# ray-project/kuberay

Measured on AMD Instinct MI355X. Metric: rayclusters_to_ready_per_sec, higher is better.
Workload: dtype bf16; 1 GPU; model=raycluster-control-plane, global_batch=2500, seq_len=4, parallelism=dp1, workers_per_cluster=3, gpus_per_worker=1, kubelet=simulated (envtest methodology; no real kubelet)

## Files before the change

### kuberay_amd/_native/build.py

```python
from __future__ import annotations

import os
import subprocess
import sys
import sysconfig
from pathlib import Path

HERE = Path(__file__).resolve().parent
GFX_ARCH = os.environ.get("PYTORCH_ROCM_ARCH", "gfx950")
HIPCC = os.environ.get("HIPCC", "/opt/rocm/bin/hipcc")


def _ext_suffix() -> str:
    return sysconfig.get_config_var("EXT_SUFFIX") or ".so"


def _pybind11_includes() -> list:
    import pybind11
    return [f"-I{pybind11.get_include()}",
            f"-I{sysconfig.get_paths()['include']}"]


def _needs_rebuild(src: Path, out: Path, *deps: Path) -> bool:
    if not out.exists():
# ... 11 lines not shown
        HIPCC, f"--offload-arch={GFX_ARCH}", "-O3", "-std=c++17",
        "-shared", "-fPIC", *_pybind11_includes(),
        str(src), "-o", str(out),
    ]
    subprocess.run(cmd, check=True)
    return out


def build_engine(force: bool = False) -> Path:
    src = HERE / "engine.cpp"
    out = HERE / f"engine{_ext_suffix()}"
    if not src.exists():
        return out
    if not force and not _needs_rebuild(src, out, HERE / "store_core.hpp",
                                        HERE / "tree_copy.hpp",
                                        HERE / "json_decode.hpp"):
        return out
    cxx = os.environ.get("CXX", "g++")
    cmd = [
        cxx, "-O3", "-std=c++17", "-shared", "-fPIC",
        *_pybind11_includes(), str(src), "-o", str(out),
    ]
    subprocess.run(cmd, check=True)
    return out


def build_all(force: bool = False) -> list:
    outs = [build_gpuhealth(force)]
    if (HERE / "engine.cpp").exists():
        outs.append(build_engine(force))
    return outs
# ... 7 lines not shown
```

### kuberay_amd/_native/engine.cpp

```cpp

#include <pybind11/pybind11.h>
#include <pybind11/stl.h>

#include <cmath>
#include <cstdio>
#include <optional>
#include <string>
#include <unordered_set>
#include <vector>

#define KUBERAY_JSON_WITH_PYTHON
#include "json_decode.hpp"
#include "store_core.hpp"
#include "tree_copy.hpp"

namespace py = pybind11;
using namespace kuberay_store;

namespace {

struct Decline {};

constexpr int kMaxDepth = 128;

struct Keys {
  PyObject *metadata, *status, *spec, *labels, *ownerReferences, *uid,
      *resourceVersion, *finalizers, *deletionTimestamp, *name, *ns, *phase,
      *podIP, *restartPolicy, *creationTimestamp, *conditions, *type,
      *containers, *containerStatuses, *state, *terminated, *clusterIP, *ports,
      *port, *nodePort;
};
Keys K;

void init_keys() {
  auto mk = [](const char* s) { return PyUnicode_InternFromString(s); };
  K.metadata = mk("metadata"); K.status = mk("status"); K.spec = mk("spec");
  K.labels = mk("labels"); K.ownerReferences = mk("ownerReferences");
  K.uid = mk("uid"); K.resourceVersion = mk("resourceVersion");
  K.finalizers = mk("finalizers");
  K.deletionTimestamp = mk("deletionTimestamp");
  K.name = mk("name"); K.ns = mk("namespace"); K.phase = mk("phase");
  K.podIP = mk("podIP"); K.restartPolicy = mk("restartPolicy");
  K.creationTimestamp = mk("creationTimestamp");
  K.conditions = mk("conditions"); K.type = mk("type");
  K.containers = mk("containers");
  K.containerStatuses = mk("containerStatuses"); K.state = mk("state");
  K.terminated = mk("terminated");
  K.clusterIP = mk("clusterIP"); K.ports = mk("ports"); K.port = mk("port");
  K.nodePort = mk("nodePort");
}


void encode_str(PyObject* s, std::string& out) {
  Py_ssize_t n = 0;
  const char* p = PyUnicode_AsUTF8AndSize(s, &n);
  if (p == nullptr) {
    PyErr_Clear();
    throw Decline{};
  }
  static const char* hex = "0123456789abcdef";
  out.push_back('"');
  const char* run = p;
  const char* end = p + n;
  for (const char* c = p; c < end; ++c) {
// ... 275 lines not shown
using ServiceViewTuple =
    std::tuple<std::string, std::string, std::string, std::vector<PortTuple>>;

Section make_section(const std::string& scratch) {
  return std::make_shared<const std::string>(scratch.data(), scratch.size());
}

py::bytes to_bytes(const Blob& b) {
  const size_t n = b.size();
  PyObject* out = PyBytes_FromStringAndSize(nullptr, static_cast<Py_ssize_t>(n));
  if (out == nullptr) throw py::error_already_set();
  b.write(PyBytes_AS_STRING(out));
  return py::reinterpret_steal<py::bytes>(out);
}

class NativeStore {
 public:
  explicit NativeStore(size_t history_capacity) : core_(history_capacity) {}

  py::object put_object(const std::string& kind, const std::string& ns,
                        const std::string& name, py::handle obj,
                        const std::optional<std::string>& event_type) {
    static thread_local std::string rest, meta_s, status_s;
    rest.clear(); meta_s.clear(); status_s.clear();
    Blob blob;
    Fields f;
    try {
      PyObject* o = obj.ptr();
      if (!PyDict_CheckExact(o)) throw Decline{};
      bool has_meta = false, has_status = false;
      Py_ssize_t pos = 0;
      PyObject *k, *v;
      while (PyDict_Next(o, &pos, &k, &v)) {
        if (!PyUnicode_CheckExact(k)) throw Decline{};
        if (PyUnicode_CompareWithASCIIString(k, "metadata") == 0) {
          encode(v, meta_s, 1);
          has_meta = true;
        } else if (PyUnicode_CompareWithASCIIString(k, "status") == 0) {
          encode(v, status_s, 1);
          has_status = true;
        } else {
          if (!rest.empty()) rest.push_back(',');
          encode_str(k, rest);
// ... 7 lines not shown
      f.rv = std::move(p.rv); f.uid = std::move(p.uid);
      f.deletion_ts = std::move(p.deletion_ts);
      f.has_finalizers = p.has_finalizers;
      extract_indexes(meta, f);
      if (kind == "Pod") {
        extract_view(o, meta, f.view);
        f.has_view = true;
      } else if (kind == "Service") {
        f.has_service_view = extract_service_view(o, meta, f.service_view);
      }
      blob.rest = make_section(rest);
      if (has_meta) blob.meta = make_section(meta_s);
      if (has_status) blob.status = make_section(status_s);
    } catch (const Decline&) {
      core_.note_fallback();
      return py::none();
    }
    core_.note_encode(true, rest.size() + meta_s.size() + status_s.size());
    const bool is_new = core_.put(kind, ns, name, std::move(blob), std::move(f),
                                  event_type ? event_type->c_str() : nullptr);
    return py::bool_(is_new);
  }

  py::object put_status(const std::string& kind, const std::string& ns,
                        const std::string& name, py::handle obj,
                        const std::optional<std::string>& event_type) {
    static thread_local std::string meta_s, status_s;
    meta_s.clear(); status_s.clear();
    Section meta_sec, status_sec;
    Peek p;
    PodViewData view;
    const bool is_pod = kind == "Pod";
    try {
      PyObject* o = obj.ptr();
      if (!PyDict_CheckExact(o)) throw Decline{};
      PyObject* meta = metadata_of(o);
      if (meta != nullptr) {
        encode(meta, meta_s, 1);
        meta_sec = make_section(meta_s);
      }
      if (PyObject* status = dget(o, K.status)) {
        encode(status, status_s, 1);
        status_sec = make_section(status_s);
      }
      extract_peek(meta, p);
      if (is_pod) extract_view(o, meta, view);
    } catch (const Decline&) {
      return py::none();
    }
    if (!core_.put_status(kind, ns, name, std::move(meta_sec),
                          std::move(status_sec), std::move(p), is_pod,
                          std::move(view),
                          event_type ? event_type->c_str() : nullptr)) {
      return py::none();
    }
    core_.note_encode(false, meta_s.size() + status_s.size());
    return py::bool_(true);
  }

  bool put(const std::string& kind, const std::string& ns,
           const std::string& name, const std::string& blob,
           const std::string& rv, const LabelList& labels,
           const std::vector<std::string>& owner_uids,
           const std::optional<PodViewData>& view,
           const std::optional<std::string>& event_type,
           const std::string& uid, bool has_finalizers,
           const std::string& deletion_ts,
           const std::optional<ServiceViewTuple>& service_view) {
    Blob b;
    b.rest = std::make_shared<const std::string>(blob);
    b.whole = true;
    Fields f;
// ... 203 lines not shown

  std::vector<int64_t> history_rvs() const { return core_.history_rvs(); }

  py::dict stats() const {
    const Stats s = core_.stats();
    py::dict d;
    d["full_encodes"] = s.full_encodes;
    d["partial_encodes"] = s.partial_encodes;
    d["bytes_encoded"] = s.bytes_encoded;
    d["blobs_assembled"] = s.blobs_assembled;
    d["bytes_assembled"] = s.bytes_assembled;
    d["fallbacks"] = s.fallbacks;
    d["history_appends"] = s.history_appends;
    d["trees_decoded"] = s.trees_decoded;
    d["decode_fallbacks"] = s.decode_fallbacks;
    return d;
  }

 private:
  StoreCore core_;
};

}

PYBIND11_MODULE(engine, m) {
  m.doc() = "kuberay-amd native object store (C++ sections + indexes + pod "
            "and Service views + watch history, native JSON encoding) and "
            "model-tree copier";
  init_keys();

  m.def("copy_configure", [](py::handle base_model) {
    return kuberay_copy::configure(base_model.ptr());
  }, py::arg("base_model"),
        "Hand the copier pydantic.BaseModel; returns whether it is enabled.");
  m.def("copy_tree", [](py::handle obj) -> py::object {
// ... 10 lines not shown
    return d;
  });

  py::class_<PodViewData>(m, "PodViewData")
      .def(py::init<>())
      .def_readwrite("name", &PodViewData::name)
      .def_readwrite("ns", &PodViewData::ns)
      .def_readwrite("phase", &PodViewData::phase)
      .def_readwrite("deletion_ts", &PodViewData::deletion_ts)
      .def_readwrite("pod_ip", &PodViewData::pod_ip)
      .def_readwrite("restart_policy", &PodViewData::restart_policy)
      .def_readwrite("creation_ts", &PodViewData::creation_ts)
      .def_readwrite("ready", &PodViewData::ready)
      .def_readwrite("terminated", &PodViewData::terminated);

  py::class_<NativeStore>(m, "NativeStore")
      .def(py::init<size_t>(), py::arg("history_capacity") = 1024)
      .def("put_object", &NativeStore::put_object, py::arg("kind"),
           py::arg("ns"), py::arg("name"), py::arg("obj"),
           py::arg("event_type") = std::nullopt)
      .def("put_status", &NativeStore::put_status, py::arg("kind"),
           py::arg("ns"), py::arg("name"), py::arg("obj"),
           py::arg("event_type") = std::nullopt)
      .def("put", &NativeStore::put, py::arg("kind"), py::arg("ns"),
           py::arg("name"), py::arg("blob"), py::arg("rv"), py::arg("labels"),
           py::arg("owner_uids"), py::arg("view") = std::nullopt,
           py::arg("event_type") = std::nullopt, py::arg("uid") = "",
           py::arg("has_finalizers") = false, py::arg("deletion_ts") = "",
           py::arg("service_view") = std::nullopt)
      .def("fetch", &NativeStore::fetch)
      .def("fetch_tree", &NativeStore::fetch_tree)
      .def("remove_tree", &NativeStore::remove_tree, py::arg("kind"),
// ... 27 lines not shown
```

### kuberay_amd/_native/store_core.hpp

```cpp
#pragma once

#include <algorithm>
#include <atomic>
#include <cstdint>
#include <cstring>
#include <memory>
#include <mutex>
#include <optional>
#include <string>
#include <tuple>
#include <unordered_map>
#include <unordered_set>
#include <utility>
#include <vector>

namespace kuberay_store {

using Section = std::shared_ptr<const std::string>;
using LabelList = std::vector<std::pair<std::string, std::string>>;

struct PodViewData {
  std::string name, ns, phase, deletion_ts, pod_ip, restart_policy, creation_ts;
  bool ready = false;
  bool terminated = false;
// ... 77 lines not shown
  PodViewData view;
  LabelList labels;
};

struct HistoryItem {
  std::string event_type;
  Blob blob;
  std::optional<int64_t> rv_override;
};

struct Stats {
  uint64_t full_encodes = 0, partial_encodes = 0, bytes_encoded = 0;
  uint64_t blobs_assembled = 0, bytes_assembled = 0;
  uint64_t fallbacks = 0, history_appends = 0;
  uint64_t trees_decoded = 0, decode_fallbacks = 0;
};

inline std::string make_key(const std::string& kind, const std::string& ns,
                            const std::string& name) {
  std::string k;
  k.reserve(kind.size() + ns.size() + name.size() + 2);
  k += kind; k += '\x1f'; k += ns; k += '\x1f'; k += name;
  return k;
}

inline std::string label_key(const std::string& kind, const std::string& k,
                             const std::string& v) {
  std::string out;
  out.reserve(kind.size() + k.size() + v.size() + 2);
  out += kind; out += '\x1f'; out += k; out += '\x1f'; out += v;
// ... 63 lines not shown
    return it->second.f.rv;
  }

  std::optional<Peek> peek(const std::string& kind, const std::string& ns,
                           const std::string& name) const {
    std::lock_guard<std::mutex> g(mu_);
    auto it = objects_.find(make_key(kind, ns, name));
    if (it == objects_.end()) return std::nullopt;
    const Fields& f = it->second.f;
    Peek p;
    p.rv = f.rv; p.uid = f.uid; p.deletion_ts = f.deletion_ts;
    p.has_finalizers = f.has_finalizers;
    return p;
  }

  bool contains(const std::string& kind, const std::string& ns,
                const std::string& name) const {
    std::lock_guard<std::mutex> g(mu_);
    return objects_.count(make_key(kind, ns, name)) != 0;
  }

  std::optional<Blob> remove(const std::string& kind, const std::string& ns,
                             const std::string& name,
                             std::optional<int64_t> event_rv = std::nullopt) {
    std::lock_guard<std::mutex> g(mu_);
    auto it = objects_.find(make_key(kind, ns, name));
    if (it == objects_.end()) return std::nullopt;
    Blob out = std::move(it->second.blob);
    index_remove(it->first, it->second);
    objects_.erase(it);
// ... 128 lines not shown

  void note_encode(bool full, size_t bytes) {
    (full ? full_encodes_ : partial_encodes_).fetch_add(1, std::memory_order_relaxed);
    bytes_encoded_.fetch_add(bytes, std::memory_order_relaxed);
  }
  void note_assembled(size_t blobs, size_t bytes) {
    blobs_assembled_.fetch_add(blobs, std::memory_order_relaxed);
    bytes_assembled_.fetch_add(bytes, std::memory_order_relaxed);
  }
  void note_fallback() { fallbacks_.fetch_add(1, std::memory_order_relaxed); }
  void note_decode(bool decoded) {
    (decoded ? trees_decoded_ : decode_fallbacks_)
        .fetch_add(1, std::memory_order_relaxed);
  }

  Stats stats() const {
    Stats s;
    s.full_encodes = full_encodes_.load(std::memory_order_relaxed);
    s.partial_encodes = partial_encodes_.load(std::memory_order_relaxed);
    s.bytes_encoded = bytes_encoded_.load(std::memory_order_relaxed);
    s.blobs_assembled = blobs_assembled_.load(std::memory_order_relaxed);
    s.bytes_assembled = bytes_assembled_.load(std::memory_order_relaxed);
    s.fallbacks = fallbacks_.load(std::memory_order_relaxed);
    s.history_appends = history_appends_.load(std::memory_order_relaxed);
    s.trees_decoded = trees_decoded_.load(std::memory_order_relaxed);
    s.decode_fallbacks = decode_fallbacks_.load(std::memory_order_relaxed);
    return s;
  }

 private:
  struct Entry {
    std::string kind, ns, name;
// ... 113 lines not shown
  mutable std::mutex mu_;
  std::unordered_map<std::string, Entry> objects_;
  std::unordered_map<std::string, std::unordered_set<std::string>> kind_index_;
  std::unordered_map<std::string, std::unordered_set<std::string>> label_index_;
  std::unordered_map<std::string, std::unordered_set<std::string>> owner_index_;

  std::vector<HistEntry> ring_;
  size_t ring_head_ = 0, ring_len_ = 0;
  int64_t base_ = 0;
  int64_t last_rv_ = 0;

  std::atomic<uint64_t> full_encodes_{0}, partial_encodes_{0}, bytes_encoded_{0};
  std::atomic<uint64_t> blobs_assembled_{0}, bytes_assembled_{0};
  std::atomic<uint64_t> fallbacks_{0}, history_appends_{0};
  std::atomic<uint64_t> trees_decoded_{0}, decode_fallbacks_{0};
};

}
```

### kuberay_amd/kube/controller.py

```python
from __future__ import annotations

import dataclasses
import logging
import threading
import traceback
from typing import Any, Dict, List, Optional, Tuple

from .store import ConflictError, InMemoryApiServer
from .workqueue import RateLimitingQueue

logger = logging.getLogger("kuberay.controller")

Request = Tuple[str, str]


@dataclasses.dataclass
class Result:
    requeue: bool = False
    requeue_after: Optional[float] = None


class Reconciler:

    def reconcile(self, request: Request) -> Result:
# ... 133 lines not shown


class Manager:

    def __init__(self, server: InMemoryApiServer):
        self.server = server
        self.controllers: List[Controller] = []
        self._watcher = None
        self._thread: Optional[threading.Thread] = None
        self._stopped = threading.Event()

    def add_controller(self, controller: Controller) -> None:
        self.controllers.append(controller)

    def _dispatch_loop(self) -> None:
        while not self._stopped.is_set():
            ev = self._watcher.next(timeout=0.5)
            if ev is None:
                continue
            event_type, obj = ev
            for c in self.controllers:
                c.observe(event_type, obj)

    def start(self) -> None:
        kinds = set()
        for c in self.controllers:
            kinds.add(c.primary_kind)
            kinds.update(c.owned_kinds)
        self._watcher = self.server.watch(kinds)
        for c in self.controllers:
            for obj in self.server.list(c.primary_kind):
                c.observe("ADDED", obj)
        self._thread = threading.Thread(target=self._dispatch_loop,
                                        name="manager-dispatch", daemon=True)
        self._thread.start()
        for c in self.controllers:
            c.start()

    def stop(self) -> None:
        self._stopped.set()
        for c in self.controllers:
            c.stop()
        if self._watcher:
# ... 13 lines not shown
```

### kuberay_amd/kube/kubelet.py

```python
from __future__ import annotations

import heapq
import itertools
import threading
import time
from typing import Callable, List, Optional, Tuple

from ..utils import constants as C
from .store import InMemoryApiServer, NotFoundError, now_iso


class SimKubelet:
    def __init__(
        self,
        server: InMemoryApiServer,
        startup_delay: float = 0.0,
        job_runtime: float = 0.05,
        gpu_gate: Optional[Callable[[dict], bool]] = None,
        executors: int = 1,
    ):
        self.server = server
        self.startup_delay = startup_delay
        self.job_runtime = job_runtime
        self.gpu_gate = gpu_gate
        self.executors = max(1, executors)
        self._ip_counter = itertools.count(1)
        self._timer_lock = threading.Condition()
        self._timers: List[Tuple[float, int, Callable[[], None]]] = []
        self._seq = 0
        self._stopped = threading.Event()
        self._threads: List[threading.Thread] = []
        self._watcher = None

    WATCHED_KINDS = ("Pod", "Job", "Gateway", "HTTPRoute")

    def start(self) -> None:
        self._watcher = self.server.watch(set(self.WATCHED_KINDS))
        for kind in self.WATCHED_KINDS:
            for obj in self.server.list(kind):
                self._on_event("ADDED", obj)
        t1 = threading.Thread(target=self._watch_loop, name="sim-kubelet-watch", daemon=True)
        self._threads = [t1]
        for i in range(self.executors):
            self._threads.append(threading.Thread(
                target=self._timer_loop, name=f"sim-kubelet-timer-{i}",
                daemon=True))
        for t in self._threads:
            t.start()

    def stop(self) -> None:
        self._stopped.set()
        if self._watcher:
# ... 158 lines not shown
```

### kuberay_amd/kube/native.py

```python
from __future__ import annotations

import json
import os
from typing import Any, Dict, List, Optional, Tuple

from .._native import engine
from .store import Key, PodView, ServiceView, compute_service_view

_dumps = json.dumps
_loads = json.loads


def _view_of(obj: Dict[str, Any]):
    status = obj.get("status") or {}
    spec = obj.get("spec") or {}
    meta = obj.get("metadata", {})
    v = engine.PodViewData()
    v.name = meta.get("name", "")
    v.ns = meta.get("namespace", "default")
    v.phase = status.get("phase") or ""
    v.deletion_ts = meta.get("deletionTimestamp") or ""
    v.pod_ip = status.get("podIP") or ""
    v.restart_policy = spec.get("restartPolicy") or ""
    v.creation_ts = meta.get("creationTimestamp") or ""
# ... 5 lines not shown
        ray_name = containers[0].get("name")
        for cs in status.get("containerStatuses") or []:
            if cs.get("name") == ray_name and (cs.get("state") or {}).get("terminated"):
                v.terminated = True
                break
    return v


class NativeBackend:
    name = "native-cpp"

    native_encode = os.environ.get("KUBERAY_STORE_NATIVE_ENCODE", "1") != "0"
    status_splice = os.environ.get("KUBERAY_STORE_STATUS_SPLICE", "1") != "0"
    native_decode = os.environ.get("KUBERAY_STORE_NATIVE_DECODE", "1") != "0"

    def __init__(self, history_limit: int = 1024) -> None:
        self._store = engine.NativeStore(history_limit)
        self._kind_counts: Dict[str, int] = {}

    def put(self, key: Key, obj: Dict[str, Any],
            event_type: Optional[str] = None) -> None:
        kind, ns, name = key
        is_new = (self._store.put_object(kind, ns, name, obj, event_type)
                  if self.native_encode else None)
        if is_new is None:
            is_new = self._put_blob(key, obj, event_type)
        if is_new:
            self._kind_counts[kind] = self._kind_counts.get(kind, 0) + 1

    def _put_blob(self, key: Key, obj: Dict[str, Any],
                  event_type: Optional[str]) -> bool:
        kind, ns, name = key
        meta = obj.get("metadata", {})
# ... 127 lines not shown
```

### kuberay_amd/kube/store.py

```python
from __future__ import annotations

import dataclasses
import threading
import time
import uuid
from collections import defaultdict, deque
from typing import Any, Dict, Iterable, List, Optional, Tuple

Key = Tuple[str, str, str]


def jsoncopy(obj):
    t = type(obj)
    if t is dict:
        return {k: jsoncopy(v) for k, v in obj.items()}
    if t is list:
        return [jsoncopy(v) for v in obj]
    return obj


class ApiError(Exception):
    def __init__(self, code: int, message: str):
        super().__init__(f"{code}: {message}")
        self.code = code
# ... 7 lines not shown

class ConflictError(ApiError):
    def __init__(self, message: str = "conflict"):
        super().__init__(409, message)


class AlreadyExistsError(ApiError):
    def __init__(self, message: str = "already exists"):
        super().__init__(409, message)


class GoneError(ApiError):

    def __init__(self, message: str = "resource version too old"):
        super().__init__(410, message)


def now_iso() -> str:
    return time.strftime("%Y-%m-%dT%H:%M:%SZ", time.gmtime())


def match_labels(labels: Optional[Dict[str, str]], selector: Optional[Dict[str, str]]) -> bool:
    if not selector:
        return True
    labels = labels or {}
    return all(labels.get(k) == v for k, v in selector.items())



@dataclasses.dataclass
# ... 217 lines not shown
class InMemoryApiServer:

    EVENT_HISTORY_LIMIT = 1024

    def __init__(self, backend=None) -> None:
        self._lock = threading.RLock()
        self._backend = backend if backend is not None else default_backend()
        self._rv = 0
        self._watchers: List["Watcher"] = []
        self._event_history: deque = deque(maxlen=self.EVENT_HISTORY_LIMIT)
        self._history_base: int = 0
        self._fast = all(hasattr(self._backend, n) for n in (
            "put_status", "peek", "history_since", "history_reset"))
        if self._fast:
            self._backend.history_reset(0, self.EVENT_HISTORY_LIMIT)

    @property
    def backend_name(self) -> str:
        return self._backend.name

    def _next_rv(self) -> str:
        self._rv += 1
        return str(self._rv)

    def _put(self, key: Key, obj: Dict[str, Any], event_type: str,
             status_only: bool = False) -> None:
        if not self._fast:
            self._backend.put(key, obj)
        elif status_only:
            self._backend.put_status(key, obj, event_type)
        else:
            self._backend.put(key, obj, event_type)

    def _notify(self, event_type: str, obj: Dict[str, Any]) -> None:
        if not self._fast:
            try:
                rv = int(obj.get("metadata", {}).get("resourceVersion") or self._rv)
            except (TypeError, ValueError):
                rv = self._rv
            if event_type == "DELETED":
                rv = self._rv
            import json as _json
            self._event_history.append(
                (rv, event_type, obj.get("kind", ""),
                 _json.dumps(obj, separators=(",", ":"))))
        for w in list(self._watchers):
            w.push(event_type, obj)

    def reset_history(self, rv: int) -> None:
        with self._lock:
            self._rv = rv
            self._history_base = rv
            self._event_history.clear()
            if self._fast:
                self._backend.history_reset(rv, self.EVENT_HISTORY_LIMIT)

    @property
    def current_rv(self) -> int:
        with self._lock:
            return self._rv
# ... 18 lines not shown
        return (obj.get("kind", ""), meta.get("namespace", "default"),
                meta.get("name", ""))

    def create(self, obj: Dict[str, Any], *, assume_owned: bool = False) -> Dict[str, Any]:
        if not assume_owned:
            obj = jsoncopy(obj)
        meta = obj.setdefault("metadata", {})
        meta.setdefault("namespace", "default")
        if not meta.get("name"):
            gen = meta.get("generateName")
            if not gen:
                raise ApiError(422, "name or generateName required")
            meta["name"] = gen + uuid.uuid4().hex[:5]
        with self._lock:
            key = self._key_of(obj)
            if self._backend.contains(key):
                raise AlreadyExistsError(f"{key} already exists")
            meta["uid"] = str(uuid.uuid4())
            meta["resourceVersion"] = self._next_rv()
            meta["generation"] = 1
            meta["creationTimestamp"] = now_iso()
            self._put(key, obj, "ADDED")
        self._notify("ADDED", obj)
        return obj

    def get(self, kind: str, namespace: str, name: str) -> Dict[str, Any]:
        with self._lock:
            obj = self._backend.fetch((kind, namespace, name))
        if obj is None:
            raise NotFoundError(f"{kind} {namespace}/{name} not found")
        return obj

    def try_get(self, kind: str, namespace: str, name: str) -> Optional[Dict[str, Any]]:
        with self._lock:
            return self._backend.fetch((kind, namespace, name))

# ... 13 lines not shown
            return self._backend.list_views(namespace, label_selector)

    def service_view(self, namespace: str, name: str) -> Optional[ServiceView]:
        fn = getattr(self._backend, "service_view", None)
        if fn is None:
            return None
        with self._lock:
            return fn(("Service", namespace, name))

    def update(self, obj: Dict[str, Any], *, subresource: Optional[str] = None,
               assume_owned: bool = False) -> Dict[str, Any]:
        if not assume_owned:
            obj = jsoncopy(obj)
        key = self._key_of(obj)
        with self._lock:
            current = self._backend.fetch(key)
            if current is None:
                raise NotFoundError(f"{key} not found")
            new_obj, finalizers_gone = self._apply_update(
                key, obj, current, subresource)
        self._notify("MODIFIED", new_obj)
        if finalizers_gone:
            self._finalize_delete(key)
        return new_obj

    def _apply_update(self, key: Key, obj: Dict[str, Any],
                      current: Dict[str, Any], subresource: Optional[str]):
        meta = obj.setdefault("metadata", {})
        rv = meta.get("resourceVersion")
        cur_meta = current["metadata"]
        if rv is not None and rv != cur_meta["resourceVersion"]:
            raise ConflictError(
                f"{key}: resourceVersion mismatch {rv} != {cur_meta['resourceVersion']}")
        if subresource == "status":
            new_obj = current
            new_obj["status"] = obj.get("status", {})
# ... 53 lines not shown
                key, merged, current, subresource)
        self._notify("MODIFIED", new_obj)
        if finalizers_gone:
            self._finalize_delete(key)
        return new_obj

    def mutate_status(self, kind: str, namespace: str, name: str,
                      fn) -> Optional[Dict[str, Any]]:
        key = (kind, namespace, name)
        with self._lock:
            obj = self._backend.fetch(key)
            if obj is None:
                return None
            if fn(obj) is False:
                return None
            new_obj, finalizers_gone = self._apply_update(
                key, obj, obj, "status")
        self._notify("MODIFIED", new_obj)
        if finalizers_gone:
            self._finalize_delete(key)
        return new_obj

    def delete(self, kind: str, namespace: str, name: str) -> None:
        key = (kind, namespace, name)
        with self._lock:
            if self._fast:
                peeked = self._backend.peek(key)
                if peeked is None:
                    raise NotFoundError(f"{kind} {namespace}/{name} not found")
                _, _, has_finalizers, deletion_ts = peeked
                if has_finalizers and deletion_ts:
                    return
                current = self._backend.fetch(key) if has_finalizers else None
            else:
                current = self._backend.fetch(key)
                if current is None:
                    raise NotFoundError(f"{kind} {namespace}/{name} not found")
                if not current["metadata"].get("finalizers"):
                    current = None
                elif current["metadata"].get("deletionTimestamp"):
                    return
            if current is not None:
                current["metadata"]["deletionTimestamp"] = now_iso()
                current["metadata"]["resourceVersion"] = self._next_rv()
                self._put(key, current, "MODIFIED")
        if current is not None:
            self._notify("MODIFIED", current)
            return
        self._finalize_delete(key)

    def _finalize_delete(self, key: Key) -> None:
        with self._lock:
            if self._fast:
                current = self._backend.remove(key, self._rv + 1)
            else:
                current = self._backend.remove(key)
            if current is None:
                return
            current["metadata"]["resourceVersion"] = self._next_rv()
            uid = current["metadata"]["uid"]
            dependents = self._backend.dependents(uid)
            self._backend.drop_owner(uid)
        self._notify("DELETED", current)
        for dep in dependents:
            try:
                self.delete(*dep)
            except NotFoundError:
                pass

    def watch(self, kinds: Optional[Iterable[str]] = None) -> "Watcher":
        w = Watcher(self, set(kinds) if kinds else None)
        with self._lock:
            self._watchers.append(w)
        return w

    def stop_watch(self, w: "Watcher") -> None:
        with self._lock:
            if w in self._watchers:
                self._watchers.remove(w)

    def count(self, kind: str) -> int:
        with self._lock:
            return self._backend.count(kind)

    def contains(self, kind: str, namespace: str, name: str) -> bool:
        with self._lock:
            return self._backend.contains((kind, namespace, name))


class Watcher:

    def __init__(self, server: InMemoryApiServer, kinds: Optional[set]):
        self._server = server
        self._kinds = kinds
        self._cond = threading.Condition()
        self._events: deque = deque()
        self._stopped = False

    def push(self, event_type: str, obj: Dict[str, Any]) -> None:
        if self._kinds is not None and obj.get("kind") not in self._kinds:
            return
        with self._cond:
            if self._stopped:
                return
            self._events.append((event_type, obj))
            self._cond.notify_all()

    def next(self, timeout: Optional[float] = None) -> Optional[Tuple[str, Dict[str, Any]]]:
        with self._cond:
            if not self._events:
                self._cond.wait(timeout)
            if self._events:
                return self._events.popleft()
            return None

    def drain(self) -> List[Tuple[str, Dict[str, Any]]]:
        with self._cond:
            events, self._events = list(self._events), deque()
            return events

    def stop(self) -> None:
        with self._cond:
            self._stopped = True
            self._cond.notify_all()
        self._server.stop_watch(self)
```

Before: 621.7 clusters/s.

## Move watch fan-out and create/status/delete verbs into native store engine

```diff
diff --git a/kuberay_amd/_native/build.py b/kuberay_amd/_native/build.py
--- a/kuberay_amd/_native/build.py
+++ b/kuberay_amd/_native/build.py
@@ -49,7 +49,8 @@
         return out
     if not force and not _needs_rebuild(src, out, HERE / "store_core.hpp",
                                         HERE / "tree_copy.hpp",
-                                        HERE / "json_decode.hpp"):
+                                        HERE / "json_decode.hpp",
+                                        HERE / "watch_hub.hpp"):
         return out
     cxx = os.environ.get("CXX", "g++")
     cmd = [
diff --git a/kuberay_amd/_native/engine.cpp b/kuberay_amd/_native/engine.cpp
--- a/kuberay_amd/_native/engine.cpp
+++ b/kuberay_amd/_native/engine.cpp
@@ -13,6 +13,7 @@
 #include "json_decode.hpp"
 #include "store_core.hpp"
 #include "tree_copy.hpp"
+#include "watch_hub.hpp"
 
 namespace py = pybind11;
 using namespace kuberay_store;
@@ -28,7 +29,7 @@
       *resourceVersion, *finalizers, *deletionTimestamp, *name, *ns, *phase,
       *podIP, *restartPolicy, *creationTimestamp, *conditions, *type,
       *containers, *containerStatuses, *state, *terminated, *clusterIP, *ports,
-      *port, *nodePort;
+      *port, *nodePort, *generation, *ADDED, *MODIFIED, *DELETED;
 };
 Keys K;
 
@@ -48,6 +49,9 @@
   K.terminated = mk("terminated");
   K.clusterIP = mk("clusterIP"); K.ports = mk("ports"); K.port = mk("port");
   K.nodePort = mk("nodePort");
+  K.generation = mk("generation");
+  K.ADDED = mk("ADDED"); K.MODIFIED = mk("MODIFIED");
+  K.DELETED = mk("DELETED");
 }
 
 
@@ -353,6 +357,148 @@
   return py::reinterpret_steal<py::bytes>(out);
 }
 
+
+struct PyEvent {
+  PyObject* type = nullptr;
+  PyObject* obj = nullptr;
+};
+using PyHub = kuberay_watch::WatchHub<PyEvent>;
+using PySub = kuberay_watch::Subscription<PyEvent>;
+using kuberay_watch::NameSet;
+
+void release_events(std::vector<PyEvent>& events) {
+  for (PyEvent& ev : events) {
+    Py_XDECREF(ev.type);
+    Py_XDECREF(ev.obj);
+  }
+  events.clear();
+}
+
+py::object event_tuple(const PyEvent& ev) {
+  PyObject* t = PyTuple_New(2);
+  if (t == nullptr) {
+    Py_DECREF(ev.type);
+    Py_DECREF(ev.obj);
+    throw py::error_already_set();
+  }
+  PyTuple_SET_ITEM(t, 0, ev.type);
+  PyTuple_SET_ITEM(t, 1, ev.obj);
+  return py::reinterpret_steal<py::object>(t);
+}
+
+std::string kind_text(PyObject* kind) {
+  if (kind != nullptr && PyUnicode_CheckExact(kind)) {
+    Py_ssize_t n = 0;
+    const char* p = PyUnicode_AsUTF8AndSize(kind, &n);
+    if (p != nullptr) return std::string(p, n);
+    PyErr_Clear();
+  }
+  return std::string("\0", 1);
+}
+
+size_t hub_publish(PyHub& hub, PyObject* type, const std::string& type_text,
+                   const std::string& kind, PyObject* obj) {
+  const size_t n = hub.publish(type_text, kind, PyEvent{type, obj});
+  for (size_t i = 0; i < n; ++i) {
+    Py_INCREF(type);
+    Py_INCREF(obj);
+  }
+  return n;
+}
+
+class WatchSubscription {
+ public:
+  explicit WatchSubscription(std::shared_ptr<PySub> sub)
+      : sub_(std::move(sub)) {}
+  WatchSubscription(const WatchSubscription&) = delete;
+  WatchSubscription& operator=(const WatchSubscription&) = delete;
+  ~WatchSubscription() { stop(); }
+
+  bool push(py::str event_type, py::handle kind, py::handle obj) {
+    const PyEvent ev{event_type.ptr(), obj.ptr()};
+    if (!sub_->offer(std::string(event_type), kind_text(kind.ptr()), ev)) {
+      return false;
+    }
+    Py_INCREF(ev.type);
+    Py_INCREF(ev.obj);
+    return true;
+  }
+
+  py::object next(std::optional<double> timeout) {
+    PyEvent ev;
+    bool got;
+    {
+      py::gil_scoped_release unlocked;
+      got = sub_->next(wait_seconds(timeout), ev);
+    }
+    if (!got) return py::none();
+    return event_tuple(ev);
+  }
+
+  py::list next_batch(std::optional<double> timeout, size_t max) {
+    std::vector<PyEvent> events;
+    {
+      py::gil_scoped_release unlocked;
+      sub_->next_batch(wait_seconds(timeout), max, events);
+    }
+    return to_list(events);
+  }
+
+  py::list drain() {
+    std::vector<PyEvent> events = sub_->drain();
+    return to_list(events);
+  }
+
+  void stop() {
+    std::vector<PyEvent> events = sub_->stop();
+    release_events(events);
+  }
+
+  size_t size() const { return sub_->size(); }
+  bool stopped() const { return sub_->stopped(); }
+  uint64_t delivered() const { return sub_->delivered(); }
+
+ private:
+  static double wait_seconds(const std::optional<double>& timeout) {
+    if (!timeout) return -1.0;
+    return *timeout > 0 ? *timeout : 0.0;
+  }
+
+  static py::list to_list(std::vector<PyEvent>& events) {
+    PyObject* out = PyList_New(static_cast<Py_ssize_t>(events.size()));
+    if (out == nullptr) {
+      release_events(events);
+      throw py::error_already_set();
+    }
+    py::list result = py::reinterpret_steal<py::list>(out);
+    for (size_t i = 0; i < events.size(); ++i) {
+      const PyEvent ev = events[i];
+      events[i] = PyEvent{};
+      try {
+        PyList_SET_ITEM(out, static_cast<Py_ssize_t>(i),
+                        event_tuple(ev).release().ptr());
+      } catch (...) {
+        release_events(events);
+        throw;
+      }
+    }
+    return result;
+  }
+
+  std::shared_ptr<PySub> sub_;
+};
+
+py::object text_object(const std::string& s) {
+  PyObject* o = PyUnicode_FromStringAndSize(s.data(),
+                                            static_cast<Py_ssize_t>(s.size()));
+  if (o == nullptr) throw py::error_already_set();
+  return py::reinterpret_steal<py::object>(o);
+}
+
+void dict_set(PyObject* d, PyObject* key, PyObject* value) {
+  if (PyDict_SetItem(d, key, value) < 0) throw py::error_already_set();
+}
+
 class NativeStore {
  public:
   explicit NativeStore(size_t history_capacity) : core_(history_capacity) {}
@@ -360,12 +506,20 @@
   py::object put_object(const std::string& kind, const std::string& ns,
                         const std::string& name, py::handle obj,
                         const std::optional<std::string>& event_type) {
+    const int r = write_tree(kind, ns, name, obj.ptr(),
+                             event_type ? event_type->c_str() : nullptr);
+    if (r < 0) return py::none();
+    return py::bool_(r == 1);
+  }
+
+  int write_tree(const std::string& kind, const std::string& ns,
+                 const std::string& name, PyObject* o,
+                 const char* event_type) {
     static thread_local std::string rest, meta_s, status_s;
     rest.clear(); meta_s.clear(); status_s.clear();
     Blob blob;
     Fields f;
     try {
-      PyObject* o = obj.ptr();
       if (!PyDict_CheckExact(o)) throw Decline{};
       bool has_meta = false, has_status = false;
       Py_ssize_t pos = 0;
@@ -403,17 +557,26 @@
       if (has_status) blob.status = make_section(status_s);
     } catch (const Decline&) {
       core_.note_fallback();
-      return py::none();
+      return -1;
     }
     core_.note_encode(true, rest.size() + meta_s.size() + status_s.size());
-    const bool is_new = core_.put(kind, ns, name, std::move(blob), std::move(f),
-                                  event_type ? event_type->c_str() : nullptr);
-    return py::bool_(is_new);
+    return core_.put(kind, ns, name, std::move(blob), std::move(f), event_type)
+               ? 1 : 0;
   }
 
   py::object put_status(const std::string& kind, const std::string& ns,
                         const std::string& name, py::handle obj,
                         const std::optional<std::string>& event_type) {
+    if (!splice_status(kind, ns, name, obj.ptr(),
+                       event_type ? event_type->c_str() : nullptr)) {
+      return py::none();
+    }
+    return py::bool_(true);
+  }
+
+  bool splice_status(const std::string& kind, const std::string& ns,
+                     const std::string& name, PyObject* o,
+                     const char* event_type) {
     static thread_local std::string meta_s, status_s;
     meta_s.clear(); status_s.clear();
     Section meta_sec, status_sec;
@@ -421,7 +584,6 @@
     PodViewData view;
     const bool is_pod = kind == "Pod";
     try {
-      PyObject* o = obj.ptr();
       if (!PyDict_CheckExact(o)) throw Decline{};
       PyObject* meta = metadata_of(o);
       if (meta != nullptr) {
@@ -435,16 +597,176 @@
       extract_peek(meta, p);
       if (is_pod) extract_view(o, meta, view);
     } catch (const Decline&) {
-      return py::none();
+      return false;
     }
     if (!core_.put_status(kind, ns, name, std::move(meta_sec),
                           std::move(status_sec), std::move(p), is_pod,
-                          std::move(view),
-                          event_type ? event_type->c_str() : nullptr)) {
+                          std::move(view), event_type)) {
+      return false;
+    }
+    core_.note_encode(false, meta_s.size() + status_s.size());
+    return true;
+  }
+
+  WatchSubscription* subscribe(std::optional<NameSet> kinds,
+                               std::optional<NameSet> event_types) {
+    return new WatchSubscription(
+        hub_->subscribe(std::move(kinds), std::move(event_types)));
+  }
+
+  size_t publish(py::str event_type, py::handle kind, py::handle obj) {
+    return hub_publish(*hub_, event_type.ptr(), std::string(event_type),
+                       kind_text(kind.ptr()), obj.ptr());
+  }
+
+
+  py::object create_object(const std::string& kind, const std::string& ns,
+                           const std::string& name, py::handle obj,
+                           py::object new_uid, int64_t rv, py::object now) {
+    core_.note_verb();
+    PyObject* o = obj.ptr();
+    if (!PyDict_CheckExact(o)) return py::none();
+    PyObject* meta = PyDict_GetItemWithError(o, K.metadata);
+    if (meta == nullptr || !PyDict_CheckExact(meta)) {
+      PyErr_Clear();
       return py::none();
     }
-    core_.note_encode(false, meta_s.size() + status_s.size());
+    if (core_.contains(kind, ns, name)) return py::bool_(false);
+    dict_set(meta, K.uid, new_uid().ptr());
+    dict_set(meta, K.resourceVersion, text_object(std::to_string(rv)).ptr());
+    dict_set(meta, K.generation, py::int_(1).ptr());
+    dict_set(meta, K.creationTimestamp, now().ptr());
+    if (write_tree(kind, ns, name, o, "ADDED") < 0) return py::str("stamped");
+    hub_publish(*hub_, K.ADDED, "ADDED", kind, o);
     return py::bool_(true);
+  }
+
+  py::object apply_status(const std::string& kind, const std::string& ns,
+                          const std::string& name, py::object obj,
+                          py::object expected_rv, int64_t new_rv,
+                          bool fetched) {
+    core_.note_verb();
+    py::object tree;
+    if (fetched) {
+      tree = std::move(obj);
+    } else {
+      if (!PyDict_CheckExact(obj.ptr())) return py::none();
+      std::optional<std::pair<Blob, Peek>> cur =
+          core_.fetch_peek(kind, ns, name);
+      if (!cur) return py::bool_(false);
+      if (cur->first.whole) return py::none();
+      if (!expected_rv.is_none()) {
+        py::object stored_rv = text_object(cur->second.rv);
+        const int differs = PyObject_RichCompareBool(
+            expected_rv.ptr(), stored_rv.ptr(), Py_NE);
+        if (differs < 0) {
+          PyErr_Clear();
+          return py::none();
+        }
+        if (differs) return stored_rv;
+      }
+      core_.note_assembled(1, cur->first.size());
+      tree = decode(cur->first);
+      if (!PyDict_CheckExact(tree.ptr())) return py::none();
+      PyObject* status = PyDict_GetItemWithError(obj.ptr(), K.status);
+      if (status == nullptr) {
+        if (PyErr_Occurred()) {
+          PyErr_Clear();
+          return py::none();
+        }
+        dict_set(tree.ptr(), K.status, py::dict().ptr());
+      } else {
+        dict_set(tree.ptr(), K.status, status);
+      }
+    }
+    PyObject* t = tree.ptr();
+    if (!PyDict_CheckExact(t)) return py::none();
+    PyObject* meta = PyDict_GetItemWithError(t, K.metadata);
+    if (meta == nullptr || !PyDict_CheckExact(meta)) {
+      PyErr_Clear();
+      return py::none();
+    }
+    bool deleting, has_finalizers;
+    try {
+      deleting = truthy(dget(meta, K.deletionTimestamp));
+      has_finalizers = truthy(dget(meta, K.finalizers));
+    } catch (const Decline&) {
+      return py::none();
+    }
+    dict_set(meta, K.resourceVersion,
+             text_object(std::to_string(new_rv)).ptr());
+    if (!splice_status(kind, ns, name, t, "MODIFIED")) return py::none();
+    hub_publish(*hub_, K.MODIFIED, "MODIFIED", kind, t);
+    return py::make_tuple(tree, deleting && !has_finalizers);
+  }
+
+  py::object delete_cascade(const std::string& kind, const std::string& ns,
+                            const std::string& name, int64_t first_rv,
+                            py::object now, py::object put_slow) {
+    core_.note_verb();
+    using KeyT = std::tuple<std::string, std::string, std::string>;
+    py::list events;
+    int64_t rv = first_rv;
+    std::vector<KeyT> stack;
+    stack.emplace_back(kind, ns, name);
+    bool root = true;
+    while (!stack.empty()) {
+      const KeyT key = std::move(stack.back());
+      stack.pop_back();
+      const std::string& k = std::get<0>(key);
+      const std::string& n = std::get<1>(key);
+      const std::string& m = std::get<2>(key);
+      std::optional<Peek> p = core_.peek(k, n, m);
+      if (!p) {
+        if (root) return py::none();
+        continue;
+      }
+      root = false;
+      if (p->has_finalizers) {
+        if (!p->deletion_ts.empty()) continue;
+        std::optional<Blob> b = core_.fetch(k, n, m);
+        if (!b) continue;
+        core_.note_assembled(1, b->size());
+        py::object tree = loaded(decode(*b));
+        py::object meta = tree[py::handle(K.metadata)];
+        meta[py::handle(K.deletionTimestamp)] = now();
+        meta[py::handle(K.resourceVersion)] = text_object(std::to_string(rv));
+        if (write_tree(k, n, m, tree.ptr(), "MODIFIED") < 0) {
+          put_slow(py::make_tuple(k, n, m), tree, py::handle(K.MODIFIED));
+        }
+        ++rv;
+        hub_publish(*hub_, K.MODIFIED, "MODIFIED", k, tree.ptr());
+        events.append(py::make_tuple(py::handle(K.MODIFIED), k, tree));
+        continue;
+      }
+      std::optional<Blob> b = core_.remove(k, n, m, rv);
+      if (!b) continue;
+      core_.note_assembled(1, b->size());
+      std::vector<KeyT> deps;
+      if (!p->uid.empty()) {
+        deps = core_.dependents(p->uid);
+        core_.drop_owner(p->uid);
+      }
+      stack.insert(stack.end(), std::make_move_iterator(deps.rbegin()),
+                   std::make_move_iterator(deps.rend()));
+      py::object tree = loaded(decode(*b));
+      tree[py::handle(K.metadata)][py::handle(K.resourceVersion)] =
+          text_object(std::to_string(rv));
+      ++rv;
+      hub_publish(*hub_, K.DELETED, "DELETED", k, tree.ptr());
+      events.append(py::make_tuple(py::handle(K.DELETED), k, tree));
+    }
+    return events;
+  }
+
+  static py::object loaded(py::object decoded) {
+    if (!PyBytes_CheckExact(decoded.ptr())) return decoded;
+    static PyObject* loads = nullptr;
+    if (loads == nullptr) {
+      loads = py::object(py::module_::import("json").attr("loads"))
+                  .release().ptr();
+    }
+    return py::handle(loads)(decoded);
   }
 
   bool put(const std::string& kind, const std::string& ns,
@@ -678,11 +1000,14 @@
     d["history_appends"] = s.history_appends;
     d["trees_decoded"] = s.trees_decoded;
     d["decode_fallbacks"] = s.decode_fallbacks;
+    d["verb_calls"] = s.verb_calls;
+    d["events_published"] = hub_->published();
     return d;
   }
 
  private:
   StoreCore core_;
+  std::shared_ptr<PyHub> hub_ = std::make_shared<PyHub>();
 };
 
 }
@@ -723,8 +1048,36 @@
       .def_readwrite("ready", &PodViewData::ready)
       .def_readwrite("terminated", &PodViewData::terminated);
 
+  py::class_<WatchSubscription>(m, "WatchSubscription")
+      .def("push", &WatchSubscription::push, py::arg("event_type"),
+           py::arg("kind"), py::arg("obj"))
+      .def("next", &WatchSubscription::next, py::arg("timeout") = std::nullopt)
+      .def("next_batch", &WatchSubscription::next_batch,
+           py::arg("timeout") = std::nullopt, py::arg("max") = 256)
+      .def("drain", &WatchSubscription::drain)
+      .def("stop", &WatchSubscription::stop)
+      .def("size", &WatchSubscription::size)
+      .def("stopped", &WatchSubscription::stopped)
+      .def("delivered", &WatchSubscription::delivered);
+
   py::class_<NativeStore>(m, "NativeStore")
       .def(py::init<size_t>(), py::arg("history_capacity") = 1024)
+      .def("subscribe", &NativeStore::subscribe,
+           py::arg("kinds") = std::nullopt,
+           py::arg("event_types") = std::nullopt,
+           py::return_value_policy::take_ownership)
+      .def("publish", &NativeStore::publish, py::arg("event_type"),
+           py::arg("kind"), py::arg("obj"))
+      .def("create_object", &NativeStore::create_object, py::arg("kind"),
+           py::arg("ns"), py::arg("name"), py::arg("obj"), py::arg("new_uid"),
+           py::arg("rv"), py::arg("now"))
+      .def("apply_status", &NativeStore::apply_status, py::arg("kind"),
+           py::arg("ns"), py::arg("name"), py::arg("obj"),
+           py::arg("expected_rv"), py::arg("new_rv"),
+           py::arg("fetched") = false)
+      .def("delete_cascade", &NativeStore::delete_cascade, py::arg("kind"),
+           py::arg("ns"), py::arg("name"), py::arg("first_rv"), py::arg("now"),
+           py::arg("put_slow"))
       .def("put_object", &NativeStore::put_object, py::arg("kind"),
            py::arg("ns"), py::arg("name"), py::arg("obj"),
            py::arg("event_type") = std::nullopt)
diff --git a/kuberay_amd/_native/store_core.hpp b/kuberay_amd/_native/store_core.hpp
--- a/kuberay_amd/_native/store_core.hpp
+++ b/kuberay_amd/_native/store_core.hpp
@@ -115,6 +115,7 @@
   uint64_t blobs_assembled = 0, bytes_assembled = 0;
   uint64_t fallbacks = 0, history_appends = 0;
   uint64_t trees_decoded = 0, decode_fallbacks = 0;
+  uint64_t verb_calls = 0;
 };
 
 inline std::string make_key(const std::string& kind, const std::string& ns,
@@ -208,6 +209,19 @@
     return p;
   }
 
+  std::optional<std::pair<Blob, Peek>> fetch_peek(
+      const std::string& kind, const std::string& ns,
+      const std::string& name) const {
+    std::lock_guard<std::mutex> g(mu_);
+    auto it = objects_.find(make_key(kind, ns, name));
+    if (it == objects_.end()) return std::nullopt;
+    const Fields& f = it->second.f;
+    Peek p;
+    p.rv = f.rv; p.uid = f.uid; p.deletion_ts = f.deletion_ts;
+    p.has_finalizers = f.has_finalizers;
+    return std::make_pair(it->second.blob, std::move(p));
+  }
+
   bool contains(const std::string& kind, const std::string& ns,
                 const std::string& name) const {
     std::lock_guard<std::mutex> g(mu_);
@@ -366,8 +380,11 @@
         .fetch_add(1, std::memory_order_relaxed);
   }
 
+  void note_verb() { verb_calls_.fetch_add(1, std::memory_order_relaxed); }
+
   Stats stats() const {
     Stats s;
+    s.verb_calls = verb_calls_.load(std::memory_order_relaxed);
     s.full_encodes = full_encodes_.load(std::memory_order_relaxed);
     s.partial_encodes = partial_encodes_.load(std::memory_order_relaxed);
     s.bytes_encoded = bytes_encoded_.load(std::memory_order_relaxed);
@@ -511,6 +528,7 @@
   std::atomic<uint64_t> blobs_assembled_{0}, bytes_assembled_{0};
   std::atomic<uint64_t> fallbacks_{0}, history_appends_{0};
   std::atomic<uint64_t> trees_decoded_{0}, decode_fallbacks_{0};
+  std::atomic<uint64_t> verb_calls_{0};
 };
 
 }
diff --git a/kuberay_amd/_native/watch_hub.hpp b/kuberay_amd/_native/watch_hub.hpp
--- /dev/null
+++ b/kuberay_amd/_native/watch_hub.hpp
@@ -0,0 +1,187 @@
+#pragma once
+
+#include <algorithm>
+#include <atomic>
+#include <chrono>
+#include <condition_variable>
+#include <cstdint>
+#include <deque>
+#include <memory>
+#include <mutex>
+#include <optional>
+#include <string>
+#include <unordered_set>
+#include <utility>
+#include <vector>
+
+namespace kuberay_watch {
+
+using NameSet = std::unordered_set<std::string>;
+
+template <class Payload>
+class Subscription {
+ public:
+  Subscription(std::optional<NameSet> kinds, std::optional<NameSet> event_types)
+      : kinds_(std::move(kinds)), event_types_(std::move(event_types)) {}
+
+  bool accepts(const std::string& event_type, const std::string& kind) const {
+    if (kinds_ && kinds_->count(kind) == 0) return false;
+    if (event_types_ && event_types_->count(event_type) == 0) return false;
+    return true;
+  }
+
+  bool offer(const std::string& event_type, const std::string& kind,
+             const Payload& payload) {
+    if (!accepts(event_type, kind)) return false;
+    bool wake;
+    {
+      std::lock_guard<std::mutex> g(mu_);
+      if (stopped_) return false;
+      queue_.push_back(payload);
+      wake = parked_ > 0;
+    }
+    if (wake) cv_.notify_one();
+    delivered_.fetch_add(1, std::memory_order_relaxed);
+    return true;
+  }
+
+  bool next(double timeout_s, Payload& out) {
+    std::unique_lock<std::mutex> g(mu_);
+    if (!wait_for_event(g, timeout_s)) return false;
+    out = std::move(queue_.front());
+    queue_.pop_front();
+    return true;
+  }
+
+  size_t next_batch(double timeout_s, size_t max, std::vector<Payload>& out) {
+    std::unique_lock<std::mutex> g(mu_);
+    if (max == 0 || !wait_for_event(g, timeout_s)) return 0;
+    const size_t n = std::min(max, queue_.size());
+    for (size_t i = 0; i < n; ++i) {
+      out.push_back(std::move(queue_.front()));
+      queue_.pop_front();
+    }
+    return n;
+  }
+
+  std::vector<Payload> drain() {
+    std::lock_guard<std::mutex> g(mu_);
+    std::vector<Payload> out(std::make_move_iterator(queue_.begin()),
+                             std::make_move_iterator(queue_.end()));
+    queue_.clear();
+    return out;
+  }
+
+  std::vector<Payload> stop() {
+    std::vector<Payload> out;
+    {
+      std::lock_guard<std::mutex> g(mu_);
+      stopped_ = true;
+      out.assign(std::make_move_iterator(queue_.begin()),
+                 std::make_move_iterator(queue_.end()));
+      queue_.clear();
+    }
+    cv_.notify_all();
+    return out;
+  }
+
+  bool stopped() const {
+    std::lock_guard<std::mutex> g(mu_);
+    return stopped_;
+  }
+
+  size_t size() const {
+    std::lock_guard<std::mutex> g(mu_);
+    return queue_.size();
+  }
+
+  uint64_t delivered() const {
+    return delivered_.load(std::memory_order_relaxed);
+  }
+
+ private:
+  bool wait_for_event(std::unique_lock<std::mutex>& g, double timeout_s) {
+    if (queue_.empty() && !stopped_ && timeout_s != 0) {
+      auto ready = [this] { return stopped_ || !queue_.empty(); };
+      ++parked_;
+      if (timeout_s < 0) {
+        cv_.wait(g, ready);
+      } else {
+        const auto span = std::chrono::duration_cast<std::chrono::nanoseconds>(
+            std::chrono::duration<double>(timeout_s));
+#if defined(__SANITIZE_THREAD__)
+        cv_.wait_until(g, std::chrono::system_clock::now() + span, ready);
+#else
+        cv_.wait_for(g, span, ready);
+#endif
+      }
+      --parked_;
+    }
+    return !stopped_ && !queue_.empty();
+  }
+
+  const std::optional<NameSet> kinds_, event_types_;
+  mutable std::mutex mu_;
+  std::condition_variable cv_;
+  std::deque<Payload> queue_;
+  int parked_ = 0;
+  bool stopped_ = false;
+  std::atomic<uint64_t> delivered_{0};
+};
+
+template <class Payload>
+class WatchHub {
+ public:
+  using Sub = Subscription<Payload>;
+
+  std::shared_ptr<Sub> subscribe(std::optional<NameSet> kinds = std::nullopt,
+                                 std::optional<NameSet> event_types =
+                                     std::nullopt) {
+    auto sub = std::make_shared<Sub>(std::move(kinds), std::move(event_types));
+    std::lock_guard<std::mutex> g(mu_);
+    prune();
+    subs_.push_back(sub);
+    return sub;
+  }
+
+  size_t publish(const std::string& event_type, const std::string& kind,
+                 const Payload& payload) {
+    size_t n = 0;
+    std::lock_guard<std::mutex> g(mu_);
+    bool any_stopped = false;
+    for (const auto& sub : subs_) {
+      if (sub->offer(event_type, kind, payload)) {
+        ++n;
+      } else if (sub->stopped()) {
+        any_stopped = true;
+      }
+    }
+    if (any_stopped) prune();
+    published_.fetch_add(1, std::memory_order_relaxed);
+    return n;
+  }
+
+  size_t subscribers() const {
+    std::lock_guard<std::mutex> g(mu_);
+    return subs_.size();
+  }
+
+  uint64_t published() const {
+    return published_.load(std::memory_order_relaxed);
+  }
+
+ private:
+  void prune() {
+    subs_.erase(std::remove_if(subs_.begin(), subs_.end(),
+                               [](const std::shared_ptr<Sub>& s) {
+                                 return s->stopped();
+                               }),
+                subs_.end());
+  }
+
+  mutable std::mutex mu_;
+  std::vector<std::shared_ptr<Sub>> subs_;
+  std::atomic<uint64_t> published_{0};
+};
+
+}
diff --git a/kuberay_amd/kube/controller.py b/kuberay_amd/kube/controller.py
--- a/kuberay_amd/kube/controller.py
+++ b/kuberay_amd/kube/controller.py
@@ -171,19 +171,25 @@
         self.controllers.append(controller)
 
     def _dispatch_loop(self) -> None:
+        routes = self._routes
+        next_batch = getattr(self._watcher, "next_batch", None)
+        if next_batch is None:
+            def next_batch(timeout):
+                ev = self._watcher.next(timeout=timeout)
+                return () if ev is None else (ev,)
         while not self._stopped.is_set():
-            ev = self._watcher.next(timeout=0.5)
-            if ev is None:
-                continue
-            event_type, obj = ev
-            for c in self.controllers:
-                c.observe(event_type, obj)
+            for event_type, obj in next_batch(timeout=0.5):
+                for c in routes.get(obj.get("kind"), ()):
+                    c.observe(event_type, obj)
 
     def start(self) -> None:
         kinds = set()
+        self._routes: Dict[str, List[Controller]] = {}
         for c in self.controllers:
             kinds.add(c.primary_kind)
             kinds.update(c.owned_kinds)
+            for kind in {c.primary_kind, *c.owned_kinds}:
+                self._routes.setdefault(kind, []).append(c)
         self._watcher = self.server.watch(kinds)
         for c in self.controllers:
             for obj in self.server.list(c.primary_kind):
diff --git a/kuberay_amd/kube/kubelet.py b/kuberay_amd/kube/kubelet.py
--- a/kuberay_amd/kube/kubelet.py
+++ b/kuberay_amd/kube/kubelet.py
@@ -35,7 +35,8 @@
     WATCHED_KINDS = ("Pod", "Job", "Gateway", "HTTPRoute")
 
     def start(self) -> None:
-        self._watcher = self.server.watch(set(self.WATCHED_KINDS))
+        self._watcher = self.server.watch(set(self.WATCHED_KINDS),
+                                          event_types={"ADDED"})
         for kind in self.WATCHED_KINDS:
             for obj in self.server.list(kind):
                 self._on_event("ADDED", obj)
diff --git a/kuberay_amd/kube/native.py b/kuberay_amd/kube/native.py
--- a/kuberay_amd/kube/native.py
+++ b/kuberay_amd/kube/native.py
@@ -43,9 +43,63 @@
     status_splice = os.environ.get("KUBERAY_STORE_STATUS_SPLICE", "1") != "0"
     native_decode = os.environ.get("KUBERAY_STORE_NATIVE_DECODE", "1") != "0"
 
+    native_watch = os.environ.get("KUBERAY_NATIVE_WATCH", "1") != "0"
+    native_verbs = os.environ.get("KUBERAY_NATIVE_VERBS", "1") != "0"
+
     def __init__(self, history_limit: int = 1024) -> None:
         self._store = engine.NativeStore(history_limit)
         self._kind_counts: Dict[str, int] = {}
+
+    def _switched(self, on: bool, name: str):
+        if not on:
+            raise AttributeError(name)
+        return getattr(self._store, name)
+
+    @property
+    def subscribe(self):
+        return self._switched(self.native_watch, "subscribe")
+
+    @property
+    def publish(self):
+        return self._switched(self.native_watch, "publish")
+
+    @property
+    def _verbs_on(self) -> bool:
+        return (self.native_verbs and self.native_encode
+                and self.status_splice and self.native_decode)
+
+    @property
+    def apply_status(self):
+        return self._switched(self._verbs_on, "apply_status")
+
+    @property
+    def create_object(self):
+        self._switched(self._verbs_on, "create_object")
+        return self._create_object
+
+    @property
+    def delete_cascade(self):
+        self._switched(self._verbs_on, "delete_cascade")
+        return self._delete_cascade
+
+    def _create_object(self, kind, ns, name, obj, new_uid, rv, now):
+        created = self._store.create_object(kind, ns, name, obj, new_uid, rv,
+                                            now)
+        if created is True:
+            self._kind_counts[kind] = self._kind_counts.get(kind, 0) + 1
+        return created
+
+    def _delete_cascade(self, kind, ns, name, first_rv, now):
+        events = self._store.delete_cascade(kind, ns, name, first_rv, now,
+                                            self.put)
+        for etype, ekind, _ in events or ():
+            if etype == "DELETED":
+                n = self._kind_counts.get(ekind, 0) - 1
+                if n > 0:
+                    self._kind_counts[ekind] = n
+                else:
+                    self._kind_counts.pop(ekind, None)
+        return events
 
     def put(self, key: Key, obj: Dict[str, Any],
             event_type: Optional[str] = None) -> None:
diff --git a/kuberay_amd/kube/store.py b/kuberay_amd/kube/store.py
--- a/kuberay_amd/kube/store.py
+++ b/kuberay_amd/kube/store.py
@@ -45,6 +45,10 @@
 
     def __init__(self, message: str = "resource version too old"):
         super().__init__(410, message)
+
+
+def _new_uid() -> str:
+    return str(uuid.uuid4())
 
 
 def now_iso() -> str:
@@ -292,6 +296,17 @@
             "put_status", "peek", "history_since", "history_reset"))
         if self._fast:
             self._backend.history_reset(0, self.EVENT_HISTORY_LIMIT)
+        self._hub = all(hasattr(self._backend, n) for n in (
+            "subscribe", "publish"))
+        self._verbs = self._fast and self._hub and all(
+            hasattr(self._backend, n) for n in (
+                "create_object", "apply_status", "delete_cascade"))
+        if self._hub:
+            self._publish = self._backend.publish
+        if self._verbs:
+            self._create_object = self._backend.create_object
+            self._apply_status = self._backend.apply_status
+            self._delete_cascade = self._backend.delete_cascade
 
     @property
     def backend_name(self) -> str:
@@ -322,6 +337,12 @@
             self._event_history.append(
                 (rv, event_type, obj.get("kind", ""),
                  _json.dumps(obj, separators=(",", ":"))))
+        if self._hub:
+            self._publish(event_type, obj.get("kind"), obj)
+        if self._watchers:
+            self._push(event_type, obj)
+
+    def _push(self, event_type: str, obj: Dict[str, Any]) -> None:
         for w in list(self._watchers):
             w.push(event_type, obj)
 
@@ -370,12 +391,28 @@
             meta["name"] = gen + uuid.uuid4().hex[:5]
         with self._lock:
             key = self._key_of(obj)
-            if self._backend.contains(key):
-                raise AlreadyExistsError(f"{key} already exists")
-            meta["uid"] = str(uuid.uuid4())
-            meta["resourceVersion"] = self._next_rv()
-            meta["generation"] = 1
-            meta["creationTimestamp"] = now_iso()
+            stamped = False
+            if self._verbs:
+                created = self._create_object(
+                    key[0], key[1], key[2], obj, _new_uid, self._rv + 1,
+                    now_iso)
+                if created is True:
+                    self._rv += 1
+                    if self._watchers:
+                        self._push("ADDED", obj)
+                    return obj
+                if created is False:
+                    raise AlreadyExistsError(f"{key} already exists")
+                stamped = created is not None
+            if stamped:
+                self._rv += 1
+            else:
+                if self._backend.contains(key):
+                    raise AlreadyExistsError(f"{key} already exists")
+                meta["uid"] = _new_uid()
+                meta["resourceVersion"] = self._next_rv()
+                meta["generation"] = 1
+                meta["creationTimestamp"] = now_iso()
             self._put(key, obj, "ADDED")
         self._notify("ADDED", obj)
         return obj
@@ -419,12 +456,32 @@
             obj = jsoncopy(obj)
         key = self._key_of(obj)
         with self._lock:
+            if self._verbs and subresource == "status":
+                rv = obj.setdefault("metadata", {}).get("resourceVersion")
+                done = self._apply_status(
+                    key[0], key[1], key[2], obj, rv, self._rv + 1)
+                if done is not None:
+                    return self._status_applied(key, done, rv)
             current = self._backend.fetch(key)
             if current is None:
                 raise NotFoundError(f"{key} not found")
             new_obj, finalizers_gone = self._apply_update(
                 key, obj, current, subresource)
         self._notify("MODIFIED", new_obj)
+        if finalizers_gone:
+            self._finalize_delete(key)
+        return new_obj
+
+    def _status_applied(self, key: Key, done, rv) -> Dict[str, Any]:
+        if done is False:
+            raise NotFoundError(f"{key} not found")
+        if type(done) is str:
+            raise ConflictError(
+                f"{key}: resourceVersion mismatch {rv} != {done}")
+        new_obj, finalizers_gone = done
+        self._rv += 1
+        if self._watchers:
+            self._push("MODIFIED", new_obj)
         if finalizers_gone:
             self._finalize_delete(key)
         return new_obj
@@ -508,6 +565,11 @@
                 return None
             if fn(obj) is False:
                 return None
+            if self._verbs:
+                done = self._apply_status(
+                    kind, namespace, name, obj, None, self._rv + 1, True)
+                if done is not None:
+                    return self._status_applied(key, done, None)
             new_obj, finalizers_gone = self._apply_update(
                 key, obj, obj, "status")
         self._notify("MODIFIED", new_obj)
@@ -518,6 +580,10 @@
     def delete(self, kind: str, namespace: str, name: str) -> None:
         key = (kind, namespace, name)
         with self._lock:
+            if self._verbs:
+                if self._cascade(key) is None:
+                    raise NotFoundError(f"{kind} {namespace}/{name} not found")
+                return
             if self._fast:
                 peeked = self._backend.peek(key)
                 if peeked is None:
@@ -543,7 +609,21 @@
             return
         self._finalize_delete(key)
 
+    def _cascade(self, key: Key):
+        events = self._delete_cascade(
+            key[0], key[1], key[2], self._rv + 1, now_iso)
+        if events:
+            self._rv += len(events)
+            if self._watchers:
+                for event_type, _, obj in events:
+                    self._push(event_type, obj)
+        return events
+
     def _finalize_delete(self, key: Key) -> None:
+        if self._verbs:
+            with self._lock:
+                self._cascade(key)
+            return
         with self._lock:
             if self._fast:
                 current = self._backend.remove(key, self._rv + 1)
@@ -562,8 +642,14 @@
             except NotFoundError:
                 pass
 
-    def watch(self, kinds: Optional[Iterable[str]] = None) -> "Watcher":
-        w = Watcher(self, set(kinds) if kinds else None)
+    def watch(self, kinds: Optional[Iterable[str]] = None,
+              event_types: Optional[Iterable[str]] = None) -> "Watcher":
+        kinds = set(kinds) if kinds else None
+        event_types = set(event_types) if event_types else None
+        if self._hub:
+            return Watcher(self, kinds, event_types,
+                           self._backend.subscribe(kinds, event_types))
+        w = Watcher(self, kinds, event_types)
         with self._lock:
             self._watchers.append(w)
         return w
@@ -584,15 +670,31 @@
 
 class Watcher:
 
-    def __init__(self, server: InMemoryApiServer, kinds: Optional[set]):
+    def __init__(self, server: InMemoryApiServer, kinds: Optional[set],
+                 event_types: Optional[set] = None, subscription=None):
         self._server = server
         self._kinds = kinds
+        self._event_types = event_types
+        if subscription is not None:
+            self._sub = subscription
+            self.next = subscription.next
+            self.next_batch = subscription.next_batch
+            self.drain = subscription.drain
+            self.stop = subscription.stop
+            return
+        self._sub = None
         self._cond = threading.Condition()
         self._events: deque = deque()
         self._stopped = False
 
     def push(self, event_type: str, obj: Dict[str, Any]) -> None:
+        if self._sub is not None:
+            self._sub.push(event_type, obj.get("kind"), obj)
+            return
         if self._kinds is not None and obj.get("kind") not in self._kinds:
+            return
+        if (self._event_types is not None
+                and event_type not in self._event_types):
             return
         with self._cond:
             if self._stopped:
@@ -608,6 +710,14 @@
                 return self._events.popleft()
             return None
 
+    def next_batch(self, timeout: Optional[float] = None,
+                   max: int = 256) -> List[Tuple[str, Dict[str, Any]]]:
+        with self._cond:
+            if not self._events and max > 0:
+                self._cond.wait(timeout)
+            events = self._events
+            return [events.popleft() for _ in range(min(max, len(events)))]
+
     def drain(self) -> List[Tuple[str, Dict[str, Any]]]:
         with self._cond:
             events, self._events = list(self._events), deque()
```

Measured after the change: 547.8 clusters/s. 11.9% lower.
